# synnada-ai/datafusion-upstream

Measured on AMD Instinct MI355X. Metric: rows/sec hash-join+agg, TPC-H SF100 Q3, higher is better.
Workload: dtype int64; 1 GPU; TPC-H SF100 Q3 (3-way hash join + group-by SUM + sort), int64 keys, Decimal128(15,2) money, resident in HBM; input_rows=765043119, parallelism=1 GPU

## Files before the change

### datafusion-upstream_amd/csrc/join.hip

```cpp
#include "join_table.h"

namespace dfgpu {
constexpr uint64_t SLOT_EMPTY = ~0ull;
constexpr uint32_t NO_SLOT = 0xFFFFFFFFu;
}
using namespace dfgpu;


namespace dfgpu {

__device__ inline bool row_selected(const uint64_t* mask, int64_t i) { return mask == nullptr || bit_get(mask, i); }

__global__ void __launch_bounds__(BLOCK) k_join_build(KeySet ks, int64_t n, const uint64_t* mask, int null_eq, int force_zero,
                                                      uint64_t* slots, uint32_t* slot_count, uint64_t cap_mask, uint32_t* row_slot,
                                                      unsigned long long* counters ) {
  int64_t i = (int64_t)blockIdx.x * BLOCK + threadIdx.x;
  if (i >= n) return;
  uint32_t my_slot = NO_SLOT;
  if (row_selected(mask, i)) {
    bool any_null; uint64_t h = keyset_hash(ks, i, 0, &any_null);
    if (force_zero) h = 0;
    if (!any_null || null_eq) {
      uint64_t tag = h >> 32, s = h & cap_mask, mine = (tag << 32) | (uint64_t)i;
      for (uint64_t step = 0; step <= cap_mask; step++) {
// ... 173 lines not shown
  if (base + WAVE * PM_ROWS <= n) probe_match_chunk<T, P, OP, HAS_MASK, HAS_VALID, true>(keys, key_valid, mask, pred, ps, n, kmin, range, bitmap, match_bits, base, lane);
  else if (base < n) probe_match_chunk<T, P, OP, HAS_MASK, HAS_VALID, false>(keys, key_valid, mask, pred, ps, n, kmin, range, bitmap, match_bits, base, lane);
}
__global__ void __launch_bounds__(BLOCK) k_probe_lookup(KeySet bks, KeySet pks, const uint32_t* rows, int64_t m, int null_eq, int force_zero,
                                                        const uint64_t* slots, const uint32_t* slot_count, uint64_t cap_mask, int unique,
                                                        uint64_t* out_build, uint32_t* out_slot, uint32_t* out_cnt, uint32_t* flags) {
  int64_t i = (int64_t)blockIdx.x * BLOCK + threadIdx.x;
  if (i >= m) return;
  int64_t j = rows[i];
  bool any_null; uint64_t h = keyset_hash(pks, j, 0, &any_null);
  if (force_zero) h = 0;
  uint64_t tag = h >> 32, s = h & cap_mask; bool found = false;
  for (uint64_t step = 0; step <= cap_mask; step++) {
    uint64_t cur = slots[s];
    if (cur == SLOT_EMPTY) break;
    if ((cur >> 32) == tag && keyset_equal(bks, (int64_t)(cur & 0xFFFFFFFFull), pks, j, null_eq != 0)) { found = true; break; }
    s = (s + 1) & cap_mask;
  }
  if (!found) { atomicOr(flags, DFGPU_FLAG_TABLE_FULL); s = 0; }
  if (unique) out_build[i] = found ? (slots[s] & 0xFFFFFFFFull) : 0;
  else { out_slot[i] = (uint32_t)s; out_cnt[i] = found ? slot_count[s] : 0; }
}
__global__ void __launch_bounds__(BLOCK) k_probe_expand(const uint32_t* rows, const uint32_t* slot_of, const uint32_t* cnt, const uint64_t* offsets, int64_t m,
                                                        const uint32_t* slot_start, const uint32_t* csr_rows, uint64_t* out_build, uint32_t* out_probe) {
  const int lane = lane_id(); const int64_t w0 = ((int64_t)blockIdx.x * BLOCK + threadIdx.x) - lane;
  if (w0 >= m) return;
  const int64_t i = w0 + lane; const bool on = i < m;
  const uint32_t c = on ? cnt[i] : 0u, st = on ? slot_start[slot_of[i]] : 0u, j = on ? rows[i] : 0u;
  const uint64_t o = on ? offsets[i] : 0ull;
  const uint64_t base = (uint64_t)__shfl((long long)o, 0, 64);
  const uint64_t rel = o - base;
  const int last = 63 - __clzll((long long)ballot64(on));
  const uint64_t total = (uint64_t)__shfl((long long)(rel + c), last, 64);
  for (uint64_t k0 = 0; k0 < total; k0 += WAVE) {
    const uint64_t k = k0 + lane;
    int lo = 0, hi = last;
#pragma unroll
    for (int step = 0; step < 6; step++) { const int mid = (lo + hi + 1) >> 1; const uint64_t r = (uint64_t)__shfl((long long)rel, mid, 64); if (r <= k) lo = mid; else hi = mid - 1; }
    const uint64_t r0 = (uint64_t)__shfl((long long)rel, lo, 64); const uint32_t s0 = (uint32_t)__shfl((int)st, lo, 64), p0 = (uint32_t)__shfl((int)j, lo, 64);
    if (k < total) { const uint32_t at = s0 + (uint32_t)(k - r0); out_build[base + k] = csr_rows ? csr_rows[at] : at; out_probe[base + k] = p0; }
  }
}
template <typename T>
__global__ void __launch_bounds__(BLOCK) k_key_minmax(const T* keys, const uint32_t* row_slot, int64_t n, long long* mn, long long* mx) {
  long long lo = INT64_MAX, hi = INT64_MIN;
  for (int64_t i = (int64_t)blockIdx.x * BLOCK + threadIdx.x; i < n; i += (int64_t)gridDim.x * BLOCK)
    if (row_slot[i] != NO_SLOT) { long long v = (long long)keys[i]; lo = v < lo ? v : lo; hi = v > hi ? v : hi; }
#pragma unroll
  for (int d = 32; d > 0; d >>= 1) { long long a = __shfl_xor(lo, d, 64), b = __shfl_xor(hi, d, 64); lo = a < lo ? a : lo; hi = b > hi ? b : hi; }
  __shared__ long long slo[BLOCK / WAVE], shi[BLOCK / WAVE];
  if (lane_id() == 0) { slo[threadIdx.x >> 6] = lo; shi[threadIdx.x >> 6] = hi; }
  __syncthreads();
  if (threadIdx.x == 0) {
    for (int w = 1; w < BLOCK / WAVE; w++) { lo = slo[w] < lo ? slo[w] : lo; hi = shi[w] > hi ? shi[w] : hi; }
    if (lo <= hi) { atomicMin(mn, lo); atomicMax(mx, hi); }
  }
}
template <typename T>
__global__ void __launch_bounds__(BLOCK) k_key_setbits(const T* keys, const uint32_t* row_slot, int64_t n, int64_t kmin, uint64_t* bitmap) {
  int64_t i = (int64_t)blockIdx.x * BLOCK + threadIdx.x;
  if (i >= n || row_slot[i] == NO_SLOT) return;
  uint64_t d = (uint64_t)((int64_t)keys[i] - kmin);
  atomicOr((unsigned long long*)&bitmap[d >> 6], 1ull << (d & 63));
}
template <typename T>
__global__ void __launch_bounds__(BLOCK) k_check_increasing(const T* keys, int64_t n, unsigned long long* out ) {
  bool bad = false, dup = false;
  for (int64_t i = (int64_t)blockIdx.x * BLOCK + threadIdx.x + 1; i < n; i += (int64_t)gridDim.x * BLOCK) { T a = keys[i - 1], b = keys[i]; bad |= b < a; dup |= a == b; }
  if (ballot64(bad) && lane_id() == 0) out[0] = 1ull;
  if (ballot64(dup) && lane_id() == 0) out[3] = 1ull;
  if (blockIdx.x == 0 && threadIdx.x == 0) { out[1] = (unsigned long long)(long long)keys[0]; out[2] = (unsigned long long)(long long)keys[n - 1]; }
}
template <typename T>
__global__ void __launch_bounds__(BLOCK) k_key_setbits_unique(const T* keys, const uint64_t* mask, const uint32_t* rows, const unsigned long long* d_count, int64_t n, int64_t kmin, uint64_t* bitmap, unsigned long long* dup, const T* ckeys = nullptr) {
  const int64_t m = rows ? (int64_t)*d_count : n;
  for (int64_t j = (int64_t)blockIdx.x * BLOCK + threadIdx.x; j < m; j += (int64_t)gridDim.x * BLOCK) {
    const int64_t i = rows ? (int64_t)rows[j] : j;
    if (!rows && mask && !bit_get(mask, i)) continue;
    const uint64_t d = (uint64_t)((int64_t)(ckeys ? ckeys[j] : keys[i]) - kmin), bit = 1ull << (d & 63);
    const unsigned long long old = atomicOr((unsigned long long*)&bitmap[d >> 6], (unsigned long long)bit);
    if (old & bit) *dup = 1ull;
  }
}
template <typename T>
__global__ void __launch_bounds__(BLOCK) k_rank_rows(const T* keys, const uint64_t* mask, const uint32_t* rows, const unsigned long long* d_count, int64_t n, int64_t kmin, const uint64_t* bitmap, const uint32_t* prefix, uint32_t* row_of_rank, const T* ckeys = nullptr) {
  const int64_t m = rows ? (int64_t)*d_count : n;
  for (int64_t j = (int64_t)blockIdx.x * BLOCK + threadIdx.x; j < m; j += (int64_t)gridDim.x * BLOCK) {
    const int64_t i = rows ? (int64_t)rows[j] : j;
    if (!rows && mask && !bit_get(mask, i)) continue;
    const uint64_t d = (uint64_t)((int64_t)(ckeys ? ckeys[j] : keys[i]) - kmin);
    row_of_rank[prefix[d >> 6] + (uint32_t)__popcll(bitmap[d >> 6] & ((1ull << (d & 63)) - 1ull))] = (uint32_t)i;
  }
}
template <typename T>
__global__ void __launch_bounds__(BLOCK) k_key_run_heads(const T* keys, int64_t n, uint64_t* heads) {
  int64_t i = (int64_t)blockIdx.x * BLOCK + threadIdx.x;
  bool h = i < n && (i == 0 || keys[i - 1] != keys[i]);
  uint64_t m = ballot64(h);
  if (lane_id() == 0 && (i >> 6) < ((n + 63) >> 6)) heads[i >> 6] = m;
}
template <typename T>
__global__ void __launch_bounds__(BLOCK) k_probe_lookup_runs(const T* pkeys, const uint32_t* rows, int64_t m, int64_t kmin, const uint64_t* bitmap, const uint32_t* prefix,
                                                             const uint32_t* run_starts, int64_t n_runs, int64_t n_build, uint32_t* out_run, uint32_t* out_cnt) {
  int64_t i = (int64_t)blockIdx.x * BLOCK + threadIdx.x;
  if (i >= m) return;
  uint64_t d = (uint64_t)((int64_t)pkeys[rows[i]] - kmin);
  uint32_t r = prefix[d >> 6] + (uint32_t)__popcll(bitmap[d >> 6] & ((1ull << (d & 63)) - 1ull));
  uint32_t st = run_starts[r], en = (int64_t)r + 1 < n_runs ? run_starts[r + 1] : (uint32_t)n_build;
  out_run[i] = r; out_cnt[i] = en - st;
}
template <typename T>
__global__ void __launch_bounds__(BLOCK) k_key_setbits_masked(const T* keys, const uint64_t* mask, int64_t n, int64_t kmin, uint64_t* bitmap) {
  int64_t i = (int64_t)blockIdx.x * BLOCK + threadIdx.x;
  int lane = lane_id();
  bool on = i < n && row_selected(mask, i);
  uint64_t d = on ? (uint64_t)((int64_t)keys[i] - kmin) : 0;
  int64_t w = on ? (int64_t)(d >> 6) : -1 - lane;
  uint64_t b = on ? 1ull << (d & 63) : 0ull;
#pragma unroll
  for (int s = 1; s < WAVE; s <<= 1) {
    uint64_t ob = __shfl_up(b, s, 64); int64_t ow = __shfl_up(w, s, 64);
    if (lane >= s && ow == w) b |= ob;
  }
  int64_t nxt = __shfl_down(w, 1, 64);
  if (on && (lane == WAVE - 1 || nxt != w)) atomicOr((unsigned long long*)&bitmap[w], (unsigned long long)b);
}
template <typename T>
__global__ void __launch_bounds__(BLOCK) k_key_setbits_rows(const T* keys, const uint32_t* rows, const unsigned long long* d_count, int64_t kmin, uint64_t* bitmap) {
  const int64_t m = (int64_t)*d_count; const int lane = lane_id();
  for (int64_t j0 = (int64_t)blockIdx.x * BLOCK; j0 < m; j0 += (int64_t)gridDim.x * BLOCK) {
    const int64_t j = j0 + threadIdx.x; const bool on = j < m;
    uint64_t d = on ? (uint64_t)((int64_t)keys[rows[j]] - kmin) : 0;
    int64_t w = on ? (int64_t)(d >> 6) : -1 - lane;
    uint64_t b = on ? 1ull << (d & 63) : 0ull;
#pragma unroll
    for (int s2 = 1; s2 < WAVE; s2 <<= 1) {
      uint64_t ob = __shfl_up(b, s2, 64); int64_t ow = __shfl_up(w, s2, 64);
      if (lane >= s2 && ow == w) b |= ob;
    }
    int64_t nxt = __shfl_down(w, 1, 64);
    if (on && (lane == WAVE - 1 || nxt != w)) atomicOr((unsigned long long*)&bitmap[w], (unsigned long long)b);
  }
}
__global__ void __launch_bounds__(BLOCK) k_popc_words(const uint64_t* words, int64_t nw, uint32_t* out) {
  int64_t i = (int64_t)blockIdx.x * BLOCK + threadIdx.x;
  if (i < nw) out[i] = (uint32_t)__popcll(words[i]);
}
constexpr int LR_ROWS = 4;
template <typename T, bool ALL, bool SEL>
__global__ void __launch_bounds__(BLOCK) k_probe_lookup_rank(const T* pkeys, const uint32_t* rows, int64_t m, int64_t kmin, const uint64_t* bitmap,
                                                             const uint32_t* prefix, const uint32_t* sel_rows, int identity, uint64_t* out_build,
                                                             const uint64_t* rows_valid = nullptr, int64_t n_probe = 0) {
  const int64_t base = (int64_t)blockIdx.x * BLOCK * LR_ROWS + threadIdx.x;
  int64_t ic[LR_ROWS]; uint64_t d[LR_ROWS], r[LR_ROWS];
#pragma unroll
  for (int q = 0; q < LR_ROWS; q++) { int64_t i = base + (int64_t)q * BLOCK; ic[q] = i < m ? i : m - 1; }
  bool live[LR_ROWS];
#pragma unroll
  for (int q = 0; q < LR_ROWS; q++) live[q] = rows_valid == nullptr || valid_at(rows_valid, ic[q]);
  if constexpr (!ALL) {
#pragma unroll
    for (int q = 0; q < LR_ROWS; q++) ic[q] = rows[ic[q]];
  }
  if (rows_valid) {
#pragma unroll
    for (int q = 0; q < LR_ROWS; q++) if (!live[q] || ic[q] >= n_probe) ic[q] = 0;
  }
#pragma unroll
  for (int q = 0; q < LR_ROWS; q++) d[q] = live[q] ? (uint64_t)((int64_t)pkeys[ic[q]] - kmin) : 0;
  if (identity) {
#pragma unroll
    for (int q = 0; q < LR_ROWS; q++) r[q] = d[q];
  } else {
    uint64_t w[LR_ROWS]; uint32_t p[LR_ROWS];
#pragma unroll
    for (int q = 0; q < LR_ROWS; q++) { w[q] = bitmap[d[q] >> 6]; p[q] = prefix[d[q] >> 6]; }
#pragma unroll
    for (int q = 0; q < LR_ROWS; q++) r[q] = p[q] + (uint32_t)__popcll(w[q] & ((1ull << (d[q] & 63)) - 1ull));
    if constexpr (SEL) {
#pragma unroll
      for (int q = 0; q < LR_ROWS; q++) r[q] = sel_rows[r[q]];
    }
  }
#pragma unroll
  for (int q = 0; q < LR_ROWS; q++) { int64_t i = base + (int64_t)q * BLOCK; if (i < m) out_build[i] = r[q]; }
}
#define DFGPU_INT_KEY_DISPATCH(TYPE, CALL)                                                                      \
  switch (TYPE) {                                                                                               \
    case DFGPU_INT8: { using T = int8_t; CALL; break; } case DFGPU_INT16: { using T = int16_t; CALL; break; }   \
    case DFGPU_INT32: case DFGPU_DATE32: { using T = int32_t; CALL; break; } case DFGPU_INT64: { using T = int64_t; CALL; break; } \
    case DFGPU_UINT8: { using T = uint8_t; CALL; break; } case DFGPU_UINT16: { using T = uint16_t; CALL; break; } \
    case DFGPU_UINT32: { using T = uint32_t; CALL; break; } default: break; }
static bool int_key_type(int32_t t) { return t == DFGPU_INT8 || t == DFGPU_INT16 || t == DFGPU_INT32 || t == DFGPU_INT64 || t == DFGPU_DATE32 || t == DFGPU_UINT8 || t == DFGPU_UINT16 || t == DFGPU_UINT32; }

__global__ void k_mark_bits_u64idx(const uint64_t* idx, const uint64_t* idx_valid, int64_t n, uint64_t* bits, int64_t nbits, uint32_t* flags) {
  int64_t i = (int64_t)blockIdx.x * blockDim.x + threadIdx.x;
  if (i >= n || !valid_at(idx_valid, i)) return;
  uint64_t r = idx[i];
  if (r >= (uint64_t)nbits) { atomicOr(flags, DFGPU_FLAG_OOB); return; }
  atomicOr((unsigned long long*)&bits[r >> 6], 1ull << (r & 63));
}
__global__ void k_mark_bits_range(const uint32_t* idx, int64_t n, int64_t lo, int64_t hi, uint64_t* bits) {
  int64_t i = (int64_t)blockIdx.x * blockDim.x + threadIdx.x;
  if (i >= n) return;
  int64_t r = idx[i];
  if (r >= lo && r < hi) atomicOr((unsigned long long*)&bits[(r - lo) >> 6], 1ull << ((r - lo) & 63));
}
__global__ void k_combine_words(const uint64_t* a, uint64_t flip, const uint64_t* b, uint64_t* out, int64_t nw) {
  int64_t i = (int64_t)blockIdx.x * blockDim.x + threadIdx.x;
  if (i < nw) out[i] = (a[i] ^ flip) & (b ? b[i] : ~0ull);
}
__global__ void k_u32_to_u64(const uint32_t* in, uint64_t* out, int64_t n, uint64_t add) {
  int64_t i = (int64_t)blockIdx.x * blockDim.x + threadIdx.x;
  if (i < n) out[i] = (uint64_t)in[i] + add;
}
__global__ void k_add_u32(uint32_t* v, int64_t n, uint32_t add) {
  int64_t i = (int64_t)blockIdx.x * blockDim.x + threadIdx.x;
  if (i < n) v[i] += add;
}

template <typename F>
static const long long* key_ranges(dfgpu_ctx* ctx, int slot, int ncols, const char* sync, F&& launch) {
  std::vector<long long> init((size_t)2 * ncols); for (int c = 0; c < ncols; c++) { init[(size_t)2 * c] = INT64_MAX; init[(size_t)2 * c + 1] = INT64_MIN; }
  HIP_CHECK(hipMemcpyAsync(ctx->d_scratch64 + slot, init.data(), init.size() * 8, hipMemcpyHostToDevice, ctx->stream));
  launch((long long*)(ctx->d_scratch64 + slot));
  KERNEL_CHECK();
  if (sync) ctx->count_sync(sync);
  fetch_to_pinned(ctx, slot, ctx->d_scratch64 + slot, init.size() * 8);
  return (const long long*)(ctx->h_pinned + slot);
}

struct PackCols { int32_t n; const void* v[MAX_KEYS]; const uint64_t* valid[MAX_KEYS]; int32_t type[MAX_KEYS]; int64_t mn[MAX_KEYS]; uint64_t range[MAX_KEYS], stride[MAX_KEYS]; };
__global__ void __launch_bounds__(BLOCK) k_cols_minmax(PackCols pc, int64_t n, long long* out ) {
  for (int c = 0; c < MAX_KEYS; c++) {
    if (c >= pc.n) break;
    long long lo = INT64_MAX, hi = INT64_MIN;
    for (int64_t i = (int64_t)blockIdx.x * BLOCK + threadIdx.x; i < n; i += (int64_t)gridDim.x * BLOCK)
      if (valid_at(pc.valid[c], i)) { long long v = key_at(pc.v[c], pc.type[c], i); lo = v < lo ? v : lo; hi = v > hi ? v : hi; }
#pragma unroll
    for (int d = 32; d > 0; d >>= 1) { long long a = __shfl_xor(lo, d, 64), b = __shfl_xor(hi, d, 64); lo = a < lo ? a : lo; hi = b > hi ? b : hi; }
    if (lane_id() == 0 && lo <= hi) { atomicMin(&out[2 * c], lo); atomicMax(&out[2 * c + 1], hi); }
  }
}
__global__ void __launch_bounds__(BLOCK) k_pack_keys(PackCols pc, int64_t n, int64_t* out, uint64_t* out_valid) {
  int64_t i = (int64_t)blockIdx.x * BLOCK + threadIdx.x;
  bool ok = i < n; uint64_t p = 0;
#pragma unroll
  for (int c = 0; c < MAX_KEYS; c++) {
    if (c >= pc.n) break;
    if (ok) {
      if (!valid_at(pc.valid[c], i)) ok = false;
      else { uint64_t d = (uint64_t)(key_at(pc.v[c], pc.type[c], i) - pc.mn[c]); if (d >= pc.range[c]) ok = false; else p += d * pc.stride[c]; }
    }
  }
  if (i < n) out[i] = ok ? (int64_t)p : 0;
  if (out_valid) { uint64_t m = ballot64(ok); if (lane_id() == 0 && (i >> 6) < ((n + 63) >> 6)) out_valid[i >> 6] = m; }
}
static PackCols pack_cols(const dfgpu_join_table* t, const dfgpu_array* const* cols) {
  PackCols pc{}; pc.n = t->pack_n;
  for (int c = 0; c < t->pack_n; c++) { pc.v[c] = cols[c]->values->ptr; pc.valid[c] = cols[c]->validity ? (const uint64_t*)cols[c]->validity->ptr : nullptr; pc.type[c] = cols[c]->type;
                                        pc.mn[c] = t->pack_min[c]; pc.range[c] = t->pack_range[c]; pc.stride[c] = t->pack_stride[c]; }
// ... 65 lines not shown
    if (lo <= hi) {
      uint64_t range = (uint64_t)hi - (uint64_t)lo + 1;
      if (range != 0 && range <= (1ull << 32) && range <= (uint64_t)n * 4096 + 65536) {
        t->bitmap = alloc_buffer(ctx, bitmap_bytes((int64_t)range), true); t->key_min = lo; t->range = range;
        DFGPU_INT_KEY_DISPATCH(key0->type, hipLaunchKernelGGL((k_key_setbits<T>), dim3(grid_for(n, BLOCK)), dim3(BLOCK), 0, ctx->stream, (const T*)kv, rs, n, (int64_t)lo, (uint64_t*)t->bitmap->ptr));
        KERNEL_CHECK();
        t->mem += (int64_t)bitmap_bytes((int64_t)range);
      } else if (range != 0 && range <= (1ull << 32)) {
        t->key_min = lo; t->range = range;
        t->lazy_row_slot = alloc_buffer(ctx, (size_t)(n + 1) * 4);
        HIP_CHECK(hipMemcpyAsync(t->lazy_row_slot->ptr, row_slot->ptr, (size_t)n * 4, hipMemcpyDeviceToDevice, ctx->stream));
      }
    }
  }
  if (!t->unique) {
    t->slot_count = alloc_buffer(ctx, cap * 4, true);
    hipLaunchKernelGGL(k_count_slots, dim3(grid_for(n, BLOCK)), dim3(BLOCK), 0, ctx->stream, (const uint32_t*)row_slot->ptr, n, (uint32_t*)t->slot_count->ptr);
    hipLaunchKernelGGL(k_fix_unslotted, dim3(grid_for(n, BLOCK)), dim3(BLOCK), 0, ctx->stream, (uint32_t*)row_slot->ptr, n, (uint32_t)cap);
    BufferPtr rows = alloc_buffer(ctx, (size_t)n * 4);
    launch_iota_u32(ctx, (uint32_t*)rows->ptr, n, 0);
    radix_sort_pairs_u32(ctx, (uint32_t*)row_slot->ptr, (uint32_t*)rows->ptr, n, bits + 1);
    t->csr_rows = rows;
    t->slot_start = alloc_buffer(ctx, cap * 4);
    HIP_CHECK(hipMemcpyAsync(t->slot_start->ptr, t->slot_count->ptr, cap * 4, hipMemcpyDeviceToDevice, ctx->stream));
    exclusive_scan_u32_inplace32(ctx, (uint32_t*)t->slot_start->ptr, (int64_t)cap, nullptr);
    t->mem += (int64_t)(cap * 8 + (size_t)n * 4);
  }
}

std::shared_ptr<const OrderStats> order_stats_measure(dfgpu_ctx* ctx, const dfgpu_array* a) {
  if (!a || a->type == DFGPU_DICTIONARY || !int_key_type(a->type) || a->validity || a->length < 1) return nullptr;
  const int64_t n = a->length; const void* kv = a->values->ptr;
  zero_scratch(ctx);
  DFGPU_INT_KEY_DISPATCH(a->type, hipLaunchKernelGGL((k_check_increasing<T>), dim3(grid_for(n, BLOCK * 8, ctx->num_cus * 8)), dim3(BLOCK), 0, ctx->stream, (const T*)kv, n, (unsigned long long*)ctx->d_scratch64));
  KERNEL_CHECK();
  ctx->count_sync("sync:rank_index_check"); fetch_to_pinned(ctx, 0, ctx->d_scratch64, 32);
  OrderStats st; st.sorted = ctx->h_pinned[0] == 0; st.repeats = ctx->h_pinned[3] != 0; st.exact = true; st.lo = (int64_t)ctx->h_pinned[1]; st.hi = (int64_t)ctx->h_pinned[2];
  order_stats_set(a, st);
  return order_stats_get(a);
}
static bool build_rank_index(dfgpu_ctx* ctx, dfgpu_join_table* t) {
  int64_t n = t->n_build;
  if (!ctx->join_rank_index || ctx->force_hash_collisions || n < 2 || t->nkeys != 1 || t->null_equals_null) return false;
  const dfgpu_array* key0 = t->keys[0];
  if (key0->type == DFGPU_DICTIONARY || !int_key_type(key0->type) || key0->validity) return false;
  const void* kv = key0->values->ptr;
  KernelTimer kt_(ctx, "join_build_rank");
  auto st = order_stats_get(key0);
  if (!st) st = order_stats_measure(ctx, key0);
  auto dense = [&](const OrderStats& s2) { const uint64_t r = (uint64_t)s2.hi - (uint64_t)s2.lo + 1; return r != 0 && r <= (1ull << 32) && r <= (uint64_t)n * 4096 + 65536; };
  if (st && st->sorted && !st->exact && !dense(*st)) st = order_stats_measure(ctx, key0);
  if (!st || !st->sorted) return false;
  const bool runs = st->repeats;
  if (runs && (t->build_mask || n > 0xFFFFFFF0ll)) return false;
  long long lo = (long long)st->lo, hi = (long long)st->hi;
  uint64_t range = (uint64_t)hi - (uint64_t)lo + 1;
  if (!dense(*st)) return false;
  const uint64_t* mk = t->build_mask ? (const uint64_t*)t->build_mask->ptr : nullptr;
  int64_t nw = (int64_t)((range + 63) / 64);
  t->key_min = lo; t->range = range;
  t->rep = runs ? JoinRep::RANK_RUNS : JoinRep::RANK; t->unique = !runs; t->rank_identity = !runs && range == (uint64_t)n;
  BufferPtr heads;
  if (runs) {
    heads = alloc_buffer(ctx, bitmap_bytes(n));
    DFGPU_INT_KEY_DISPATCH(key0->type, hipLaunchKernelGGL((k_key_run_heads<T>), dim3(grid_for(n, BLOCK)), dim3(BLOCK), 0, ctx->stream, (const T*)kv, n, (uint64_t*)heads->ptr));
    KERNEL_CHECK();
    mk = (const uint64_t*)heads->ptr;
  }
  if (t->rank_identity && mk) t->bitmap = t->build_mask;
  else {
    t->bitmap = alloc_buffer(ctx, bitmap_bytes((int64_t)range)); t->mem += (int64_t)bitmap_bytes((int64_t)range);
    HIP_CHECK(hipMemsetAsync(t->bitmap->ptr, t->rank_identity ? 0xFF : 0, bitmap_bytes((int64_t)range), ctx->stream));
  }
  if (!t->rank_identity) {
    if (mk && !runs && n <= 0xFFFFFFF0ll) {
      t->sel_rows = mask_to_indices_uncounted(ctx, mk, n, ctx->d_scratch64 + 15); t->mem += t->sel_rows->length * 4;
      DFGPU_INT_KEY_DISPATCH(key0->type, hipLaunchKernelGGL((k_key_setbits_rows<T>), dim3(grid_for(n, BLOCK, ctx->num_cus * 16)), dim3(BLOCK), 0, ctx->stream, (const T*)kv, (const uint32_t*)t->sel_rows->values->ptr,
                                                            (const unsigned long long*)(ctx->d_scratch64 + 15), (int64_t)lo, (uint64_t*)t->bitmap->ptr));
    } else {
      DFGPU_INT_KEY_DISPATCH(key0->type, hipLaunchKernelGGL((k_key_setbits_masked<T>), dim3(grid_for(n, BLOCK)), dim3(BLOCK), 0, ctx->stream, (const T*)kv, mk, n, (int64_t)lo, (uint64_t*)t->bitmap->ptr));
      if (mk) { t->sel_rows = mask_to_indices_impl(ctx, mk, n); t->mem += t->sel_rows->length * 4; }
    }
    KERNEL_CHECK();
    t->rank_prefix = alloc_buffer(ctx, (size_t)nw * 4);
    hipLaunchKernelGGL(k_popc_words, dim3(grid_for(nw, BLOCK)), dim3(BLOCK), 0, ctx->stream, (const uint64_t*)t->bitmap->ptr, nw, (uint32_t*)t->rank_prefix->ptr);
    exclusive_scan_u32_inplace32(ctx, (uint32_t*)t->rank_prefix->ptr, nw, nullptr);
    KERNEL_CHECK();
    t->mem += nw * 4;
  }
  return true;
}

template <typename T>
__global__ void __launch_bounds__(BLOCK) k_key_minmax_masked(const T* keys, const uint64_t* valid, const uint64_t* mask, int64_t n, long long* mn, long long* mx, const uint32_t* rows = nullptr, const unsigned long long* d_count = nullptr) {
  long long lo = INT64_MAX, hi = INT64_MIN;
  if (rows) {
    const int64_t m = (int64_t)*d_count;
    for (int64_t j = (int64_t)blockIdx.x * BLOCK + threadIdx.x; j < m; j += (int64_t)gridDim.x * BLOCK) { const int64_t i = rows[j]; if (valid_at(valid, i)) { long long v = (long long)keys[i]; lo = v < lo ? v : lo; hi = v > hi ? v : hi; } }
  } else
  for (int64_t i = (int64_t)blockIdx.x * BLOCK + threadIdx.x; i < n; i += (int64_t)gridDim.x * BLOCK)
    if (row_selected(mask, i) && valid_at(valid, i)) { long long v = (long long)keys[i]; lo = v < lo ? v : lo; hi = v > hi ? v : hi; }
#pragma unroll
  for (int d = 32; d > 0; d >>= 1) { long long a = __shfl_xor(lo, d, 64), b = __shfl_xor(hi, d, 64); lo = a < lo ? a : lo; hi = b > hi ? b : hi; }
  __shared__ long long slo[BLOCK / WAVE], shi[BLOCK / WAVE];
  if (lane_id() == 0) { slo[threadIdx.x >> 6] = lo; shi[threadIdx.x >> 6] = hi; }
  __syncthreads();
  if (threadIdx.x == 0) {
    for (int w = 1; w < BLOCK / WAVE; w++) { lo = slo[w] < lo ? slo[w] : lo; hi = shi[w] > hi ? shi[w] : hi; }
    if (lo <= hi) { atomicMin(mn, lo); atomicMax(mx, hi); }
  }
}
template <typename T>
__global__ void __launch_bounds__(BLOCK) k_key_gather_minmax(const T* keys, const uint32_t* rows, const unsigned long long* d_count, T* ckeys, long long* mn, long long* mx) {
  const int64_t m = (int64_t)*d_count; long long lo = INT64_MAX, hi = INT64_MIN;
  for (int64_t j0 = ((int64_t)blockIdx.x * BLOCK) * 4 + threadIdx.x; j0 < m; j0 += (int64_t)gridDim.x * BLOCK * 4) {
    T k[4]; bool on[4];
#pragma unroll
    for (int q = 0; q < 4; q++) { const int64_t j = j0 + (int64_t)q * BLOCK; on[q] = j < m; k[q] = on[q] ? keys[rows[j]] : (T)0; }
#pragma unroll
    for (int q = 0; q < 4; q++) if (on[q]) { ckeys[j0 + (int64_t)q * BLOCK] = k[q]; const long long v = (long long)k[q]; lo = v < lo ? v : lo; hi = v > hi ? v : hi; }
  }
#pragma unroll
  for (int d = 32; d > 0; d >>= 1) { long long a = __shfl_xor(lo, d, 64), b = __shfl_xor(hi, d, 64); lo = a < lo ? a : lo; hi = b > hi ? b : hi; }
  __shared__ long long slo[BLOCK / WAVE], shi[BLOCK / WAVE];
  if (lane_id() == 0) { slo[threadIdx.x >> 6] = lo; shi[threadIdx.x >> 6] = hi; }
  __syncthreads();
  if (threadIdx.x == 0) {
    for (int w = 1; w < BLOCK / WAVE; w++) { lo = slo[w] < lo ? slo[w] : lo; hi = shi[w] > hi ? shi[w] : hi; }
    if (lo <= hi) { atomicMin(mn, lo); atomicMax(mx, hi); }
  }
}
static bool build_rank_index_unsorted(dfgpu_ctx* ctx, dfgpu_join_table* t) {
  const int64_t n = t->n_build;
  if (!ctx->join_rank_index || !ctx->join_rank_index_unsorted || ctx->force_hash_collisions || n < 2 || n > 0xFFFFFFF0ll || t->nkeys != 1 || t->null_equals_null) return false;
  const dfgpu_array* key0 = t->keys[0];
  if (key0->type == DFGPU_DICTIONARY || !int_key_type(key0->type) || key0->validity) return false;
  KernelTimer kt_(ctx, "join_build_rank");
  const uint64_t* mk = t->build_mask ? (const uint64_t*)t->build_mask->ptr : nullptr;
  ArrayHolder list; const uint32_t* rl = nullptr; const unsigned long long* dcount = (const unsigned long long*)(ctx->d_scratch64 + 15);
  if (mk) { list.a = mask_to_indices_uncounted(ctx, mk, n, ctx->d_scratch64 + 15); rl = (const uint32_t*)list.get()->values->ptr; }
  const int lgrid = grid_for(n, BLOCK, ctx->num_cus * 16);
  BufferPtr ck; const void* ckp = nullptr;
  long long lo, hi;
  if (rl) {
    ck = alloc_buffer(ctx, (size_t)n * type_width(key0->type) + 16); ckp = ck->ptr;
    const long long* mm = key_ranges(ctx, 4, 1, "sync:rank_index_range", [&](long long* w) {
      DFGPU_INT_KEY_DISPATCH(key0->type, hipLaunchKernelGGL((k_key_gather_minmax<T>), dim3(grid_for(n, BLOCK * 4, ctx->num_cus * 4)), dim3(BLOCK), 0, ctx->stream, (const T*)key0->values->ptr, rl, dcount, (T*)ck->ptr,
                                                            w, w + 1)); });
    lo = mm[0]; hi = mm[1];
  } else selected_key_range(ctx, t, "sync:rank_index_range", &lo, &hi);
  t->have_minmax = true; t->sel_min = lo; t->sel_max = hi;
  if (lo > hi) return false;
  const uint64_t range = (uint64_t)hi - (uint64_t)lo + 1;
  if (range == 0 || range > (1ull << 32) || range > (uint64_t)n * 256 + 65536) return false;
  const int64_t nw = (int64_t)((range + 63) / 64);
  BufferPtr bitmap = alloc_buffer(ctx, bitmap_bytes((int64_t)range));
  HIP_CHECK(hipMemsetAsync(bitmap->ptr, 0, bitmap_bytes((int64_t)range), ctx->stream));
  HIP_CHECK(hipMemsetAsync(ctx->d_scratch64 + 6, 0, 8, ctx->stream));
  DFGPU_INT_KEY_DISPATCH(key0->type, hipLaunchKernelGGL((k_key_setbits_unique<T>), dim3(lgrid), dim3(BLOCK), 0, ctx->stream, (const T*)key0->values->ptr, mk, rl, dcount, n, (int64_t)lo, (uint64_t*)bitmap->ptr,
                                                        (unsigned long long*)(ctx->d_scratch64 + 6), (const T*)ckp));
  BufferPtr prefix = alloc_buffer(ctx, (size_t)nw * 4);
  hipLaunchKernelGGL(k_popc_words, dim3(grid_for(nw, BLOCK)), dim3(BLOCK), 0, ctx->stream, (const uint64_t*)bitmap->ptr, nw, (uint32_t*)prefix->ptr);
  exclusive_scan_u32_inplace32(ctx, (uint32_t*)prefix->ptr, nw, ctx->d_scratch64 + 7);
  KERNEL_CHECK();
  const uint64_t* hsc = read_scratch_range(ctx, 6, 2);
  ctx->count_sync("sync:rank_index_unique");
  if (hsc[0] != 0) return false;
  const int64_t nsel = (int64_t)hsc[1];
  ArrayHolder rows(new_fixed(ctx, DFGPU_UINT32, nsel));
  DFGPU_INT_KEY_DISPATCH(key0->type, hipLaunchKernelGGL((k_rank_rows<T>), dim3(lgrid), dim3(BLOCK), 0, ctx->stream, (const T*)key0->values->ptr, mk, rl, dcount, n, (int64_t)lo, (const uint64_t*)bitmap->ptr,
                                                        (const uint32_t*)prefix->ptr, (uint32_t*)rows.get()->values->ptr, (const T*)ckp));
  KERNEL_CHECK();
  t->key_min = lo; t->range = range; t->rep = JoinRep::RANK; t->unique = true; t->rank_identity = false;
  t->bitmap = bitmap; t->rank_prefix = prefix; t->sel_rows = rows.release();
  t->mem += (int64_t)bitmap_bytes((int64_t)range) + nw * 4 + nsel * 4;
  return true;
}
void selected_key_range(dfgpu_ctx* ctx, const dfgpu_join_table* t, const char* sync, long long* lo, long long* hi) {
  const dfgpu_array* key0 = t->keys[0]; const int64_t n = t->n_build;
  const long long* mm = key_ranges(ctx, 4, 1, sync, [&](long long* w) {
    DFGPU_INT_KEY_DISPATCH(key0->type, hipLaunchKernelGGL((k_key_minmax_masked<T>), dim3(grid_for(n, BLOCK * 8, ctx->num_cus * 4)), dim3(BLOCK), 0, ctx->stream, (const T*)key0->values->ptr,
                                                          key0->validity ? (const uint64_t*)key0->validity->ptr : nullptr, t->build_mask ? (const uint64_t*)t->build_mask->ptr : nullptr, n, w, w + 1)); });
  *lo = mm[0]; *hi = mm[1];
}

static bool rank_lookup_ok(const dfgpu_join_table* t, const dfgpu_array* const* probe_keys, int32_t nkeys) {
  return t->rep == JoinRep::RANK && !t->pack_n && nkeys == 1 && probe_keys[0]->type == t->keys[0]->type && !probe_keys[0]->validity;
}
static void lookup_rank(dfgpu_ctx* ctx, const dfgpu_join_table* t, const dfgpu_array* pk, const uint32_t* rows, const uint64_t* rows_valid, int64_t m, bool all, uint64_t* out_build) {
  if (!m) return;
  KernelTimer kt_(ctx, "k_probe_lookup_rank");
  const bool sel = t->sel_rows != nullptr;
#define LR(ALL, SEL) DFGPU_INT_KEY_DISPATCH(pk->type, hipLaunchKernelGGL((k_probe_lookup_rank<T, ALL, SEL>), dim3(grid_for(m, BLOCK * LR_ROWS)), dim3(BLOCK), 0, ctx->stream, (const T*)pk->values->ptr, rows, m, t->key_min, \
                                                          (const uint64_t*)t->bitmap->ptr, t->rank_prefix ? (const uint32_t*)t->rank_prefix->ptr : nullptr, \
                                                          sel ? (const uint32_t*)t->sel_rows->values->ptr : nullptr, t->rank_identity ? 1 : 0, out_build, rows_valid, pk->length))
  if (all && sel) { LR(true, true); } else if (all) { LR(true, false); } else if (sel) { LR(false, true); } else { LR(false, false); }
#undef LR
  KERNEL_CHECK();
}
struct ProbePred { const dfgpu_array* col = nullptr; int op = 0; int64_t scalar = 0; };
static bool probe_pred_ok(const dfgpu_join_table* t, const dfgpu_array* pk, const ProbePred& pp) {
  auto w48 = [](int32_t ty) { return ty == DFGPU_INT32 || ty == DFGPU_DATE32 || ty == DFGPU_INT64; };
  return pp.col && pp.op >= DFGPU_OP_EQ && pp.op <= DFGPU_OP_GTEQ && w48(pp.col->type) && !pp.col->validity && pp.col->length == pk->length && w48(pk->type) && !pk->validity &&
         pk->type == t->keys[0]->type && (t->bitmap || (t->lazy_row_slot && t->range <= (uint64_t)pk->length * 16));
}
static const void* pair_aligned(dfgpu_ctx* ctx, const dfgpu_array* a, int64_t n, BufferPtr& keep) {
  const void* p = a->values->ptr; const size_t w = (size_t)type_width(a->type);
  if ((uintptr_t)p % (2 * w)) { keep = alloc_buffer(ctx, (size_t)n * w); HIP_CHECK(hipMemcpyAsync(keep->ptr, p, (size_t)n * w, hipMemcpyDeviceToDevice, ctx->stream)); p = keep->ptr; }
  return p;
}
template <typename T, typename P>
static void launch_probe_fused(dfgpu_ctx* ctx, int op, dim3 grid, const T* keys, const uint64_t* mk, const P* pred, P ps, int64_t n, int64_t kmin, uint64_t range, const uint64_t* bitmap, uint64_t* match_bits) {
  switch (op) {
#define PF_CASE(OP) case OP: if (mk) hipLaunchKernelGGL((k_probe_match_bitmap<T, P, OP, true, false>), grid, dim3(BLOCK), 0, ctx->stream, keys, (const uint64_t*)nullptr, mk, pred, ps, n, kmin, range, bitmap, match_bits); \
                             else hipLaunchKernelGGL((k_probe_match_bitmap<T, P, OP, false, false>), grid, dim3(BLOCK), 0, ctx->stream, keys, (const uint64_t*)nullptr, mk, pred, ps, n, kmin, range, bitmap, match_bits); break;
    PF_CASE(DFGPU_OP_EQ) PF_CASE(DFGPU_OP_NEQ) PF_CASE(DFGPU_OP_LT) PF_CASE(DFGPU_OP_LTEQ) PF_CASE(DFGPU_OP_GT) PF_CASE(DFGPU_OP_GTEQ)
#undef PF_CASE
    default: fail(DFGPU_INTERNAL, "fused probe: operator %d", op);
  }
}
static bool match_bits_by_bitmap(dfgpu_ctx* ctx, const dfgpu_join_table* t, const dfgpu_array* pk, int64_t n, const uint64_t* mk, uint64_t* match_bits, const ProbePred& pp = ProbePred()) {
  const dfgpu_array* key0 = t->keys[0];
  if (pk->type != key0->type) return false;
  if (t->lazy_row_slot && t->range <= (uint64_t)n * 16) {
    KernelTimer kt_(ctx, "join_build_bitmap");
    t->bitmap = alloc_buffer(ctx, bitmap_bytes((int64_t)t->range), true); t->mem += (int64_t)bitmap_bytes((int64_t)t->range);
    DFGPU_INT_KEY_DISPATCH(key0->type, hipLaunchKernelGGL((k_key_setbits<T>), dim3(grid_for(t->n_build, BLOCK)), dim3(BLOCK), 0, ctx->stream, (const T*)key0->values->ptr,
                                                          (const uint32_t*)t->lazy_row_slot->ptr, t->n_build, t->key_min, (uint64_t*)t->bitmap->ptr));
    KERNEL_CHECK();
    t->lazy_row_slot.reset();
  }
  if (!t->bitmap) return false;
  KernelTimer kt_(ctx, "k_probe_match_bitmap");
  const dim3 grid(grid_for(n, BLOCK * PM_ROWS));
  const uint64_t* kvp = pk->validity ? (const uint64_t*)pk->validity->ptr : nullptr;
  BufferPtr aligned_keys, aligned_pred; const void* kptr = pair_aligned(ctx, pk, n, aligned_keys);
  const uint64_t* bm = (const uint64_t*)t->bitmap->ptr;
  if (pp.op) {
    const void* pptr = pair_aligned(ctx, pp.col, n, aligned_pred);
    const bool k8 = pk->type == DFGPU_INT64, p8 = pp.col->type == DFGPU_INT64;
    if (k8 && p8) launch_probe_fused<int64_t, int64_t>(ctx, pp.op, grid, (const int64_t*)kptr, mk, (const int64_t*)pptr, pp.scalar, n, t->key_min, t->range, bm, match_bits);
    else if (k8) launch_probe_fused<int64_t, int32_t>(ctx, pp.op, grid, (const int64_t*)kptr, mk, (const int32_t*)pptr, (int32_t)pp.scalar, n, t->key_min, t->range, bm, match_bits);
    else if (p8) launch_probe_fused<int32_t, int64_t>(ctx, pp.op, grid, (const int32_t*)kptr, mk, (const int64_t*)pptr, pp.scalar, n, t->key_min, t->range, bm, match_bits);
    else launch_probe_fused<int32_t, int32_t>(ctx, pp.op, grid, (const int32_t*)kptr, mk, (const int32_t*)pptr, (int32_t)pp.scalar, n, t->key_min, t->range, bm, match_bits);
    return true;
  }
#define PM_LAUNCH(HM, HV) DFGPU_INT_KEY_DISPATCH(pk->type, hipLaunchKernelGGL((k_probe_match_bitmap<T, T, 0, HM, HV>), grid, dim3(BLOCK), 0, ctx->stream, (const T*)kptr, \
                                                          kvp, mk, (const T*)nullptr, (T)0, n, t->key_min, t->range, bm, match_bits))
  if (mk && kvp) { PM_LAUNCH(true, true); } else if (mk) { PM_LAUNCH(true, false); } else if (kvp) { PM_LAUNCH(false, true); } else { PM_LAUNCH(false, false); }
#undef PM_LAUNCH
  return true;
}
static BufferPtr match_bits_by_hash(dfgpu_ctx* ctx, const dfgpu_join_table* t, const dfgpu_array* const* probe_keys, int32_t nkeys, const KeySet& pks, int64_t n, const uint64_t* mk, uint64_t* match_bits) {
  if (!t->slots) build_hash_table(ctx, t, false);
  KernelTimer kt_(ctx, "k_probe_match_hash");
  auto plain8 = [](const dfgpu_array* a) { return (a->type == DFGPU_INT64 || a->type == DFGPU_UINT64) && !a->validity; };
  bool fast_hash = (nkeys == 1 || nkeys == 2) && !t->null_equals_null && !ctx->force_hash_collisions && t->n_build > 0;
  for (int c = 0; c < nkeys && fast_hash; c++) fast_hash = plain8(probe_keys[c]) && plain8(t->keys[(size_t)c]);
// ... 288 lines not shown
```

Before: 266.0 billion rows/s.

## Use per-64-byte-block rank prefix instead of per-word prefix for rank joins

Rank-based join lookups now keep one prefix count per 8-word (512-bit) block of the key bitmap instead of one per 64-bit word. The rank of a key is the block prefix plus popcounts over the block's words, read as one 64-byte line. This shrinks the prefix array eightfold so it is more likely to stay in cache, and turns two scattered random reads per lookup into one bitmap line plus a small prefix read. In exchange each lookup does up to eight popcounts and wider loads, rows per thread in the probe kernel drop from 4 to 2, and the bitmap allocation may need padding to a 64-byte multiple to avoid reading past its end.

```diff
diff --git a/datafusion-upstream_amd/csrc/join.hip b/datafusion-upstream_amd/csrc/join.hip
--- a/datafusion-upstream_amd/csrc/join.hip
+++ b/datafusion-upstream_amd/csrc/join.hip
@@ -279,6 +279,38 @@
     if (old & bit) *dup = 1ull;
   }
 }
+constexpr int RANK_BLOCK_WORDS = 8;
+struct RankBlock { ulonglong2 w[RANK_BLOCK_WORDS / 2]; uint32_t p; };
+__device__ inline RankBlock rank_block_load(const uint64_t* bitmap, const uint32_t* prefix, uint64_t d) {
+  RankBlock rb; const ulonglong2* line = (const ulonglong2*)bitmap + (d >> 9) * (RANK_BLOCK_WORDS / 2);
+#pragma unroll
+  for (int k = 0; k < RANK_BLOCK_WORDS / 2; k++) rb.w[k] = line[k];
+  rb.p = prefix[d >> 9];
+  return rb;
+}
+__device__ inline uint32_t rank_block_rank(const RankBlock& rb, uint64_t d) {
+  const int wi = (int)(d >> 6) & (RANK_BLOCK_WORDS - 1); const uint64_t low = (1ull << (d & 63)) - 1ull;
+  uint32_t r = rb.p;
+#pragma unroll
+  for (int k = 0; k < RANK_BLOCK_WORDS; k++) {
+    const uint64_t w = (k & 1) ? rb.w[k >> 1].y : rb.w[k >> 1].x;
+    r += (uint32_t)__popcll(w & (k < wi ? ~0ull : (k == wi ? low : 0ull)));
+  }
+  return r;
+}
+__device__ inline uint32_t rank_of_bit(const uint64_t* bitmap, const uint32_t* prefix, uint64_t d) { return rank_block_rank(rank_block_load(bitmap, prefix, d), d); }
+__global__ void __launch_bounds__(BLOCK) k_popc_blocks(const uint64_t* words, int64_t nw, int64_t nblocks, uint32_t* out) {
+  const int64_t b = (int64_t)blockIdx.x * BLOCK + threadIdx.x;
+  if (b >= nblocks) return;
+  const ulonglong2* line = (const ulonglong2*)words + b * (RANK_BLOCK_WORDS / 2);
+  ulonglong2 w[RANK_BLOCK_WORDS / 2];
+#pragma unroll
+  for (int k = 0; k < RANK_BLOCK_WORDS / 2; k++) w[k] = line[k];
+  const int64_t w0 = b * RANK_BLOCK_WORDS; uint32_t c = 0;
+#pragma unroll
+  for (int k = 0; k < RANK_BLOCK_WORDS / 2; k++) c += (uint32_t)__popcll(w0 + 2 * k < nw ? w[k].x : 0ull) + (uint32_t)__popcll(w0 + 2 * k + 1 < nw ? w[k].y : 0ull);
+  out[b] = c;
+}
 template <typename T>
 __global__ void __launch_bounds__(BLOCK) k_rank_rows(const T* keys, const uint64_t* mask, const uint32_t* rows, const unsigned long long* d_count, int64_t n, int64_t kmin, const uint64_t* bitmap, const uint32_t* prefix, uint32_t* row_of_rank, const T* ckeys = nullptr) {
   const int64_t m = rows ? (int64_t)*d_count : n;
@@ -286,7 +318,7 @@
     const int64_t i = rows ? (int64_t)rows[j] : j;
     if (!rows && mask && !bit_get(mask, i)) continue;
     const uint64_t d = (uint64_t)((int64_t)(ckeys ? ckeys[j] : keys[i]) - kmin);
-    row_of_rank[prefix[d >> 6] + (uint32_t)__popcll(bitmap[d >> 6] & ((1ull << (d & 63)) - 1ull))] = (uint32_t)i;
+    row_of_rank[rank_of_bit(bitmap, prefix, d)] = (uint32_t)i;
   }
 }
 template <typename T>
@@ -302,7 +334,7 @@
   int64_t i = (int64_t)blockIdx.x * BLOCK + threadIdx.x;
   if (i >= m) return;
   uint64_t d = (uint64_t)((int64_t)pkeys[rows[i]] - kmin);
-  uint32_t r = prefix[d >> 6] + (uint32_t)__popcll(bitmap[d >> 6] & ((1ull << (d & 63)) - 1ull));
+  uint32_t r = rank_of_bit(bitmap, prefix, d);
   uint32_t st = run_starts[r], en = (int64_t)r + 1 < n_runs ? run_starts[r + 1] : (uint32_t)n_build;
   out_run[i] = r; out_cnt[i] = en - st;
 }
@@ -339,11 +371,7 @@
     if (on && (lane == WAVE - 1 || nxt != w)) atomicOr((unsigned long long*)&bitmap[w], (unsigned long long)b);
   }
 }
-__global__ void __launch_bounds__(BLOCK) k_popc_words(const uint64_t* words, int64_t nw, uint32_t* out) {
-  int64_t i = (int64_t)blockIdx.x * BLOCK + threadIdx.x;
-  if (i < nw) out[i] = (uint32_t)__popcll(words[i]);
-}
-constexpr int LR_ROWS = 4;
+constexpr int LR_ROWS = 2;
 template <typename T, bool ALL, bool SEL>
 __global__ void __launch_bounds__(BLOCK) k_probe_lookup_rank(const T* pkeys, const uint32_t* rows, int64_t m, int64_t kmin, const uint64_t* bitmap,
                                                              const uint32_t* prefix, const uint32_t* sel_rows, int identity, uint64_t* out_build,
@@ -369,11 +397,11 @@
 #pragma unroll
     for (int q = 0; q < LR_ROWS; q++) r[q] = d[q];
   } else {
-    uint64_t w[LR_ROWS]; uint32_t p[LR_ROWS];
-#pragma unroll
-    for (int q = 0; q < LR_ROWS; q++) { w[q] = bitmap[d[q] >> 6]; p[q] = prefix[d[q] >> 6]; }
-#pragma unroll
-    for (int q = 0; q < LR_ROWS; q++) r[q] = p[q] + (uint32_t)__popcll(w[q] & ((1ull << (d[q] & 63)) - 1ull));
+    RankBlock rb[LR_ROWS];
+#pragma unroll
+    for (int q = 0; q < LR_ROWS; q++) rb[q] = rank_block_load(bitmap, prefix, d[q]);
+#pragma unroll
+    for (int q = 0; q < LR_ROWS; q++) r[q] = rank_block_rank(rb[q], d[q]);
     if constexpr (SEL) {
 #pragma unroll
       for (int q = 0; q < LR_ROWS; q++) r[q] = sel_rows[r[q]];
@@ -605,11 +633,12 @@
       if (mk) { t->sel_rows = mask_to_indices_impl(ctx, mk, n); t->mem += t->sel_rows->length * 4; }
     }
     KERNEL_CHECK();
-    t->rank_prefix = alloc_buffer(ctx, (size_t)nw * 4);
-    hipLaunchKernelGGL(k_popc_words, dim3(grid_for(nw, BLOCK)), dim3(BLOCK), 0, ctx->stream, (const uint64_t*)t->bitmap->ptr, nw, (uint32_t*)t->rank_prefix->ptr);
-    exclusive_scan_u32_inplace32(ctx, (uint32_t*)t->rank_prefix->ptr, nw, nullptr);
+    const int64_t nblk = (nw + RANK_BLOCK_WORDS - 1) / RANK_BLOCK_WORDS;
+    t->rank_prefix = alloc_buffer(ctx, (size_t)nblk * 4);
+    hipLaunchKernelGGL(k_popc_blocks, dim3(grid_for(nblk, BLOCK)), dim3(BLOCK), 0, ctx->stream, (const uint64_t*)t->bitmap->ptr, nw, nblk, (uint32_t*)t->rank_prefix->ptr);
+    exclusive_scan_u32_inplace32(ctx, (uint32_t*)t->rank_prefix->ptr, nblk, nullptr);
     KERNEL_CHECK();
-    t->mem += nw * 4;
+    t->mem += nblk * 4;
   }
   return true;
 }
@@ -682,9 +711,10 @@
   HIP_CHECK(hipMemsetAsync(ctx->d_scratch64 + 6, 0, 8, ctx->stream));
   DFGPU_INT_KEY_DISPATCH(key0->type, hipLaunchKernelGGL((k_key_setbits_unique<T>), dim3(lgrid), dim3(BLOCK), 0, ctx->stream, (const T*)key0->values->ptr, mk, rl, dcount, n, (int64_t)lo, (uint64_t*)bitmap->ptr,
                                                         (unsigned long long*)(ctx->d_scratch64 + 6), (const T*)ckp));
-  BufferPtr prefix = alloc_buffer(ctx, (size_t)nw * 4);
-  hipLaunchKernelGGL(k_popc_words, dim3(grid_for(nw, BLOCK)), dim3(BLOCK), 0, ctx->stream, (const uint64_t*)bitmap->ptr, nw, (uint32_t*)prefix->ptr);
-  exclusive_scan_u32_inplace32(ctx, (uint32_t*)prefix->ptr, nw, ctx->d_scratch64 + 7);
+  const int64_t nblk = (nw + RANK_BLOCK_WORDS - 1) / RANK_BLOCK_WORDS;
+  BufferPtr prefix = alloc_buffer(ctx, (size_t)nblk * 4);
+  hipLaunchKernelGGL(k_popc_blocks, dim3(grid_for(nblk, BLOCK)), dim3(BLOCK), 0, ctx->stream, (const uint64_t*)bitmap->ptr, nw, nblk, (uint32_t*)prefix->ptr);
+  exclusive_scan_u32_inplace32(ctx, (uint32_t*)prefix->ptr, nblk, ctx->d_scratch64 + 7);
   KERNEL_CHECK();
   const uint64_t* hsc = read_scratch_range(ctx, 6, 2);
   ctx->count_sync("sync:rank_index_unique");
@@ -696,7 +726,7 @@
   KERNEL_CHECK();
   t->key_min = lo; t->range = range; t->rep = JoinRep::RANK; t->unique = true; t->rank_identity = false;
   t->bitmap = bitmap; t->rank_prefix = prefix; t->sel_rows = rows.release();
-  t->mem += (int64_t)bitmap_bytes((int64_t)range) + nw * 4 + nsel * 4;
+  t->mem += (int64_t)bitmap_bytes((int64_t)range) + nblk * 4 + nsel * 4;
   return true;
 }
 void selected_key_range(dfgpu_ctx* ctx, const dfgpu_join_table* t, const char* sync, long long* lo, long long* hi) {
```

Measured after the change: 272.9 billion rows/s, median of 6. 2.6% higher.
